# Xharlie/BtcDet

Hardware: AMD Instinct MI355X
Metric: scenes/s fwd+bwd KITTI-Car bs=2/GPU (BtcDet hot path) (higher is better)
Workload: dtype f32

## Files before the change

btcdet_amd/csrc/conv_wgrad_x.hip:

```cpp
#include <type_traits>
#include <utility>

#include "conv_tile.h"

typedef short s16x4 __attribute__((ext_vector_type(4)));
typedef short s16x8 __attribute__((ext_vector_type(8)));
typedef unsigned u32x4 __attribute__((ext_vector_type(4)));

namespace {

constexpr int TMX = 64;
#define X_RECORDS 0xFFFFFF00u
#define X_ABSENT 0xFFFFFFF0u

template <int RS>
__device__ __forceinline__ bf16x8 frag_tr(const char* p) {
  typedef __attribute__((address_space(3))) s16x4* lds_p;
  const s16x4 a = __builtin_amdgcn_ds_read_tr16_b64_v4i16((lds_p)p);
  const s16x4 b = __builtin_amdgcn_ds_read_tr16_b64_v4i16((lds_p)(p + 16 * RS));
  const s16x8 v = __builtin_shufflevector(a, b, 0, 1, 2, 3, 4, 5, 6, 7);
  return __builtin_bit_cast(bf16x8, v);
}

template <int N, typename F, int... I>
__device__ __forceinline__ void static_for_impl(F&& f, std::integer_sequence<int, I...>) {
  (f(std::integral_constant<int, I>{}), ...);
}
template <int N, typename F>
__device__ __forceinline__ void static_for(F&& f) {
  static_for_impl<N>(f, std::make_integer_sequence<int, N>{});
}

template <int MT, int NT, int KB, int PH, int MODE, int DEPTH>
__global__ __launch_bounds__(256) void conv_wgrad_x(const void* __restrict__ gsrc, const void* __restrict__ csrc,
                                                    const int32_t* __restrict__ nbr, const int32_t* __restrict__ order, int n_rows, int K,
                                                    int Cg_all, int Cc_all, float* __restrict__ part, int swap) {
  constexpr int Cg = MT * 16, Cc = NT * 16;
  const int n_cblk = (Cc_all + Cc - 1) / Cc;
  const int cg0 = ((int)blockIdx.z / n_cblk) * Cg, cc0 = ((int)blockIdx.z % n_cblk) * Cc;
  constexpr int NPL = MODE ? 3 : 1;
  constexpr int RS = Cg * 2 + 16;
  constexpr int IMG = TMX * RS;
  constexpr int ITEM = KB * NPL * IMG;
  constexpr int TPP = KB * MT * NT / 4;
  static_assert(KB * MT * NT % 4 == 0, "phase tiles must split evenly over the 4 waves");
  static_assert(4 % NT == 0, "a wave's tiles must share one column block");
  constexpr int NOFF = PH * KB;
  constexpr int NV = (TMX * NOFF + 255) / 256;
  extern __shared__ __attribute__((aligned(16))) char smem[];
  char* As = smem;
  constexpr int RING = (DEPTH == 2 && PH == 1) ? 4 : 3;
  int32_t* s_nbr = (int32_t*)(As + 2 * ITEM);
  constexpr int RROW = DEPTH == 2 ? RING + 1 : RING;
  int32_t* s_row = s_nbr + RING * TMX * NOFF;

  const int tid = threadIdx.x, lane = tid & 63, wave = tid >> 6, g4 = lane >> 4, t16 = lane & 15;
  const int kg0 = blockIdx.y * NOFF;
  const int n_tiles = (n_rows + TMX - 1) / TMX;
  const int nt_wg = ((int)blockIdx.x < n_tiles) ? (n_tiles - 1 - (int)blockIdx.x) / (int)gridDim.x + 1 : 0;
  const int bcol = cc0 + (wave % NT) * 16 + t16;
  const bool bvalid = bcol < Cc_all;
  const int lane_off = (4 * g4 + (t16 >> 2)) * RS + (t16 & 3) * 8;

  constexpr int NC = MODE ? 3 : 1;
  f32x4 acc[NC][PH * TPP];
#pragma unroll
  for (int c = 0; c < NC; ++c)
#pragma unroll
    for (int t = 0; t < PH * TPP; ++t) acc[c][t] = (f32x4){0.f, 0.f, 0.f, 0.f};

  const __amdgpu_buffer_rsrc_t rg = __builtin_amdgcn_make_buffer_rsrc((void*)gsrc, 0, X_RECORDS, 0x00020000);
  const __amdgpu_buffer_rsrc_t rc = __builtin_amdgcn_make_buffer_rsrc((void*)csrc, 0, X_RECORDS, 0x00020000);
  int nv[NV], nrow = -1;
  auto load_map = [&](int i) {
    const int row0 = (blockIdx.x + i * gridDim.x) * TMX;
    if (tid < TMX) nrow = (row0 + tid < n_rows) ? (order ? order[row0 + tid] : row0 + tid) : -1;
#pragma unroll
    for (int u = 0; u < NV; ++u) {
      const int e = u * 256 + tid, r = e / NOFF, o = e - r * NOFF;
      int v = -1;
      if (e < TMX * NOFF && row0 + r < n_rows && kg0 + o < K) {
        const int gr = order ? order[row0 + r] : row0 + r;
        v = nbr[(long long)gr * K + kg0 + o];
      }
      nv[u] = v;
    }
  };
  auto store_map = [&](int i) {
    int32_t* dn = s_nbr + (i % RING) * TMX * NOFF;
#pragma unroll
    for (int u = 0; u < NV; ++u) {
      const int e = u * 256 + tid;
      if (e < TMX * NOFF) dn[e] = nv[u];
    }
    if (tid < TMX) s_row[(i % RROW) * TMX + tid] = nrow;
  };

  auto load_rows = [&](int i) {
    const int row0 = (blockIdx.x + i * gridDim.x) * TMX;
    if (tid < TMX) nrow = (row0 + tid < n_rows) ? (order ? order[row0 + tid] : row0 + tid) : -1;
  };
  auto store_rows = [&](int i) {
    if (tid < TMX) s_row[(i % RROW) * TMX + tid] = nrow;
  };
  auto load_map2 = [&](int i) {
    const int32_t* rw = s_row + (i % RROW) * TMX;
#pragma unroll
    for (int u = 0; u < NV; ++u) {
      const int e = u * 256 + tid, r = e / NOFF, o = e - r * NOFF;
      int v = -1;
      if (e < TMX * NOFF && kg0 + o < K) {
        const int gr = rw[r];
        if (gr >= 0) v = nbr[(long long)gr * K + kg0 + o];
      }
      nv[u] = v;
    }
  };
  auto store_map2 = [&](int i) {
    int32_t* dn = s_nbr + (i % RING) * TMX * NOFF;
#pragma unroll
    for (int u = 0; u < NV; ++u) {
      const int e = u * 256 + tid;
      if (e < TMX * NOFF) dn[e] = nv[u];
    }
  };

  float bnf[MODE ? 16 : 1];
  unsigned short bnh[MODE ? 1 : 16];
  bf16x8 bh[2], bm[MODE ? 2 : 1], bl[MODE ? 2 : 1];
  auto load_b = [&](int i) {
    const int32_t* rows = s_row + (i % RROW) * TMX + 4 * g4;
    int gr[16];
#pragma unroll
    for (int u = 0; u < 16; ++u) gr[u] = rows[(u >> 2) * 16 + (u & 3)];
#pragma unroll
    for (int u = 0; u < 16; ++u) {
      const unsigned off = (gr[u] >= 0 && bvalid) ? ((unsigned)gr[u] * (unsigned)Cc_all + (unsigned)bcol) * (MODE ? 4u : 2u) : X_ABSENT;
      if (MODE) bnf[u] = __uint_as_float(__builtin_amdgcn_raw_buffer_load_b32(rc, off, 0, 0));
      else bnh[u] = __builtin_amdgcn_raw_buffer_load_b16(rc, off, 0, 0);
    }
  };
  auto take_b = [&]() {
#pragma unroll
    for (int s = 0; s < 2; ++s) {
      uint4 h, m, l;
      if (MODE) {
        btc_split3(bnf[8 * s + 0], bnf[8 * s + 1], h.x, m.x, l.x);
        btc_split3(bnf[8 * s + 2], bnf[8 * s + 3], h.y, m.y, l.y);
        btc_split3(bnf[8 * s + 4], bnf[8 * s + 5], h.z, m.z, l.z);
        btc_split3(bnf[8 * s + 6], bnf[8 * s + 7], h.w, m.w, l.w);
        bm[s] = __builtin_bit_cast(bf16x8, m);
        bl[s] = __builtin_bit_cast(bf16x8, l);
      } else {
        h.x = (unsigned)bnh[8 * s + 0] | ((unsigned)bnh[8 * s + 1] << 16);
        h.y = (unsigned)bnh[8 * s + 2] | ((unsigned)bnh[8 * s + 3] << 16);
        h.z = (unsigned)bnh[8 * s + 4] | ((unsigned)bnh[8 * s + 5] << 16);
        h.w = (unsigned)bnh[8 * s + 6] | ((unsigned)bnh[8 * s + 7] << 16);
      }
      bh[s] = __builtin_bit_cast(bf16x8, h);
    }
  };

  constexpr int UPR = MODE ? MT * 4 : MT * 2;
  constexpr int NU = (KB * TMX * UPR + 255) / 256;
  uint4 gq[DEPTH][NU];
  auto load_g = [&](int i, int p, auto set_c) {
    constexpr int SET = decltype(set_c)::value;
    const int32_t* mp = s_nbr + (i % RING) * TMX * NOFF + p * KB;
    int jj[NU];
#pragma unroll
    for (int u = 0; u < NU; ++u) {
      const int e = u * 256 + tid, r = (e / UPR) % TMX, kb = e / (UPR * TMX);
      jj[u] = (e < KB * TMX * UPR) ? mp[r * NOFF + kb] : -1;
    }
#pragma unroll
    for (int u = 0; u < NU; ++u) {
      const int c = (u * 256 + tid) % UPR;
      const unsigned off = jj[u] >= 0 ? ((unsigned)jj[u] * (unsigned)Cg_all + (unsigned)cg0) * (MODE ? 4u : 2u) + (unsigned)c * 16u : X_ABSENT;
      const u32x4 v = __builtin_amdgcn_raw_buffer_load_b128(rg, off, 0, 0);
      gq[SET][u] = make_uint4(v.x, v.y, v.z, v.w);
    }
  };
  auto store_g = [&](int buf, auto set_c) {
    constexpr int SET = decltype(set_c)::value;
    char* A = As + buf * ITEM;
#pragma unroll
    for (int u = 0; u < NU; ++u) {
      const int e = u * 256 + tid, c = e % UPR, r = (e / UPR) % TMX, kb = e / (UPR * TMX);
      if (e < KB * TMX * UPR) {
        char* d = A + kb * NPL * IMG + r * RS;
        if (MODE) {
          uint2 h, m, l;
          btc_split3(__uint_as_float(gq[SET][u].x), __uint_as_float(gq[SET][u].y), h.x, m.x, l.x);
          btc_split3(__uint_as_float(gq[SET][u].z), __uint_as_float(gq[SET][u].w), h.y, m.y, l.y);
          *reinterpret_cast<uint2*>(d + c * 8) = h;
          *reinterpret_cast<uint2*>(d + IMG + c * 8) = m;
          *reinterpret_cast<uint2*>(d + 2 * IMG + c * 8) = l;
        } else {
          *reinterpret_cast<uint4*>(d + c * 16) = gq[SET][u];
        }
      }
    }
  };

  typedef std::integral_constant<int, 0> Set0;
  typedef std::integral_constant<int, DEPTH - 1> Set1;
  if (nt_wg > 0 && DEPTH == 1) {
    load_map(0);
    store_map(0);
    if (nt_wg > 1) {
      load_map(1);
      store_map(1);
    }
    __syncthreads();
    load_b(0);
    load_g(0, 0, Set0{});
  }
  if (nt_wg > 0 && DEPTH == 2) {
    for (int j = 0; j < RROW - 1 && j < nt_wg; ++j) {
      load_rows(j);
      store_rows(j);
    }
    __syncthreads();
    for (int j = 0; j < RING - 1 && j < nt_wg; ++j) {
      load_map2(j);
      store_map2(j);
    }
    __syncthreads();
    load_b(0);
    load_g(0, 0, Set0{});
    if (PH > 1) load_g(0, 1, Set1{});
    else if (nt_wg > 1) load_g(1, 0, Set1{});
  }
  int buf = 0;
  auto products = [&](auto p_c) {
    constexpr int p = decltype(p_c)::value;
    constexpr int STEPS = 2 * TPP;
    const char* A = As + buf * ITEM + lane_off;
    bf16x8 fh[2], fm[MODE ? 2 : 1], fl[MODE ? 2 : 1];
    auto read_step = [&](int t, int w) {
      const int q = t >> 1, s2 = t & 1, l = q * 4 + wave;
      const int mt = (l / NT) % MT, kb = l / (NT * MT);
      const char* ap = A + kb * NPL * IMG + mt * 32 + 32 * s2 * RS;
      fh[w] = frag_tr<RS>(ap);
      if (MODE) {
        fm[MODE ? w : 0] = frag_tr<RS>(ap + IMG);
        fl[MODE ? w : 0] = frag_tr<RS>(ap + 2 * IMG);
      }
    };
    read_step(0, 0);
#pragma unroll
    for (int t = 0; t < STEPS; ++t) {
      const int q = t >> 1, s2 = t & 1, w = t & 1;
      if (t + 1 < STEPS) read_step(t + 1, w ^ 1);
      const bf16x8 ah = fh[w];
      if (MODE) {
        const bf16x8 am = fm[MODE ? w : 0], al = fl[MODE ? w : 0];
        f32x4 c2 = acc[NC - 1][p * TPP + q], c1 = acc[NC > 1 ? 1 : 0][p * TPP + q], c0 = acc[0][p * TPP + q];
        c2 = __builtin_amdgcn_mfma_f32_16x16x32_bf16(al, bh[s2], c2, 0, 0, 0);
        c1 = __builtin_amdgcn_mfma_f32_16x16x32_bf16(am, bh[s2], c1, 0, 0, 0);
        c0 = __builtin_amdgcn_mfma_f32_16x16x32_bf16(ah, bh[s2], c0, 0, 0, 0);
        c2 = __builtin_amdgcn_mfma_f32_16x16x32_bf16(ah, bl[MODE ? s2 : 0], c2, 0, 0, 0);
        c1 = __builtin_amdgcn_mfma_f32_16x16x32_bf16(ah, bm[MODE ? s2 : 0], c1, 0, 0, 0);
        c2 = __builtin_amdgcn_mfma_f32_16x16x32_bf16(am, bm[MODE ? s2 : 0], c2, 0, 0, 0);
        acc[NC - 1][p * TPP + q] = c2;
        acc[NC > 1 ? 1 : 0][p * TPP + q] = c1;
        acc[0][p * TPP + q] = c0;
      } else {
        acc[0][p * TPP + q] = __builtin_amdgcn_mfma_f32_16x16x32_bf16(ah, bh[s2], acc[0][p * TPP + q], 0, 0, 0);
      }
    }
  };
  if (DEPTH == 1) {
    for (int i = 0; i < nt_wg; ++i) {
      static_for<PH>([&](auto p_c) {
        constexpr int p = decltype(p_c)::value;
        store_g(buf, Set0{});
        if (p == 0) take_b();
        if (PH > 1 ? (p == 1 && i + 2 < nt_wg) : (i >= 1 && i + 1 < nt_wg)) store_map(PH > 1 ? i + 2 : i + 1);
        __syncthreads();
        if (p + 1 < PH) {
          load_g(i, p + 1, Set0{});
        } else if (i + 1 < nt_wg) {
          load_b(i + 1);
          load_g(i + 1, 0, Set0{});
        }
        if (PH > 1 ? (p == 0 && i + 2 < nt_wg) : (i + 2 < nt_wg)) load_map(i + 2);
        products(p_c);
        buf ^= 1;
      });
    }
  } else if (PH > 1) {
    for (int i = 0; i < nt_wg; ++i) {
      static_for<PH>([&](auto p_c) {
        constexpr int p = decltype(p_c)::value;
        typedef std::integral_constant<int, (p & 1) ? DEPTH - 1 : 0> Set;
        store_g(buf, Set{});
        if (p == 0) take_b();
        if (p == 1 && i + 2 < nt_wg) store_map2(i + 2);
        if (p == 1 && i + 3 < nt_wg) store_rows(i + 3);
        __syncthreads();
        if (p == PH - 2 && i + 1 < nt_wg) load_b(i + 1);
        if (p == 0 && i + 3 < nt_wg) load_rows(i + 3);
        if (p == 0 && i + 2 < nt_wg) load_map2(i + 2);
        if (p + 2 < PH) load_g(i, p + 2, Set{});
        else if (i + 1 < nt_wg) load_g(i + 1, p + 2 - PH, Set{});
        products(p_c);
        buf ^= 1;
      });
    }
  } else {
    auto tile = [&](int i, auto set_c) {
      store_g(buf, set_c);
      take_b();
      if (i >= 1 && i + 2 < nt_wg) store_map2(i + 2);
      if (i >= 1 && i + 3 < nt_wg) store_rows(i + 3);
      __syncthreads();
      if (i + 1 < nt_wg) load_b(i + 1);
      if (i + 4 < nt_wg) load_rows(i + 4);
      if (i + 3 < nt_wg) load_map2(i + 3);
      if (i + 2 < nt_wg) load_g(i + 2, 0, set_c);
      products(std::integral_constant<int, 0>{});
      buf ^= 1;
    };
    for (int i = 0; i < nt_wg; i += 2) {
      tile(i, Set0{});
      if (i + 1 < nt_wg) tile(i + 1, Set1{});
    }
  }
  float* P = part + (size_t)blockIdx.x * K * Cg_all * Cc_all;
#pragma unroll
  for (int p = 0; p < PH; ++p)
#pragma unroll
    for (int q = 0; q < TPP; ++q) {
      const int l = q * 4 + wave;
      const int nt = l % NT, mt = (l / NT) % MT, kb = l / (NT * MT);
      const int k = kg0 + p * KB + kb;
      const int co = cc0 + nt * 16 + t16;
      if (k >= K || co >= Cc_all) continue;
#pragma unroll
      for (int r = 0; r < 4; ++r) {
        const int ci = cg0 + mt * 16 + g4 * 4 + r;
        float v = acc[0][p * TPP + q][r];
        if (MODE) v = v + (acc[NC > 1 ? 1 : 0][p * TPP + q][r] + acc[NC - 1][p * TPP + q][r]);
        if (!swap) P[((size_t)k * Cg_all + ci) * Cc_all + co] = v;
        else P[((size_t)k * Cc_all + co) * Cg_all + ci] = v;
      }
    }
}

template <int MT, int NT, int KB, int PH, int MODE, int DEPTH>
size_t lds_x() {
  constexpr int NPL = MODE ? 3 : 1;
  constexpr int RING = (DEPTH == 2 && PH == 1) ? 4 : 3;
  constexpr int RROW = DEPTH == 2 ? RING + 1 : RING;
  return (size_t)2 * KB * NPL * TMX * (MT * 32 + 16) + (size_t)(RING * TMX * PH * KB + RROW * TMX) * sizeof(int32_t);
}

template <int MT, int NT, int KB, int PH, int MODE, int DEPTH>
void launch_x(dim3 grid, hipStream_t stream, const void* g, const void* c, const int32_t* map, const int32_t* ord, int rows, int K, int cg_all,
              int cc_all, float* part, int swap) {
  static BtcPerDeviceOnce once;
  btc_once_per_device(once, [] {
    (void)hipFuncSetAttribute((const void*)conv_wgrad_x<MT, NT, KB, PH, MODE, DEPTH>, hipFuncAttributeMaxDynamicSharedMemorySize, 160 * 1024);
  });
  conv_wgrad_x<MT, NT, KB, PH, MODE, DEPTH><<<grid, 256, lds_x<MT, NT, KB, PH, MODE, DEPTH>(), stream>>>(g, c, map, ord, rows, K, cg_all, cc_all, part, swap);
}

struct XShape {
  int mt, nt, kb, ph;
};
const XShape X_BF16[] = {{4, 4, 1, 4}, {4, 2, 1, 8}, {2, 4, 2, 4}, {3, 2, 2, 4}, {2, 2, 2, 8}, {2, 1, 2, 8}, {1, 2, 4, 4}, {1, 1, 4, 4}};
const XShape X_SPLIT[] = {{4, 4, 1, 2}, {4, 2, 1, 4}, {2, 4, 2, 2}, {3, 2, 2, 2}, {2, 2, 2, 4}, {2, 1, 2, 8}, {1, 2, 2, 8}};

const XShape* find_shape(int mode, int cg_all, int cc_all) {
  if (cg_all <= 0 || cc_all <= 0 || (cg_all & 15)) return nullptr;
  const XShape* tab = mode ? X_SPLIT : X_BF16;
  const int n = mode ? (int)(sizeof(X_SPLIT) / sizeof(XShape)) : (int)(sizeof(X_BF16) / sizeof(XShape));
  const int nt_want = cc_all <= 16 ? 1 : (cc_all <= 32 ? 2 : 4);
  for (int nt = nt_want; nt >= 1; nt >>= 1)
    for (int i = 0; i < n; ++i) {
      if (tab[i].nt != nt) continue;
      const int cg = tab[i].mt * 16;
      if (cg_all % cg != 0 || (tab[i].mt == 3 && cg_all != 48)) continue;
      return tab + i;
    }
  return nullptr;
}

}

bool btc_wgrad_x_supported(int mode, int K, int cg, int cc) {
  if (K > 64 || K < 1) return false;
  return find_shape(mode, cg, cc) != nullptr;
}

int btc_wgrad_x_plan(int mode, int rows, int K, int cg, int cc, int* S, int* ph, int* z) {
  const XShape* sh = find_shape(mode, cg, cc);
  const int t_wgs = btc_tune_get(BTC_TUNE_WGRAD_WGS);
  const int wgs = t_wgs ? t_wgs : 512;
  const int n_tiles = btc_cdiv(rows, TMX);
  const int nz = (cg / (sh->mt * 16)) * btc_cdiv(cc, sh->nt * 16);
  int p = sh->ph;
  if (p > 1 && (long long)n_tiles * btc_cdiv(K, sh->kb * p) * nz < 3LL * wgs) p >>= 1;
  const int groups = btc_cdiv(K, sh->kb * p);
  int s = wgs / (groups * nz);
  if (s > n_tiles / 2) s = n_tiles / 2;
  if (s < 1) s = 1;
  *S = s;
  *ph = p;
  if (z) *z = nz;
  return groups;
}

int btc_launch_wgrad_x(int mode, const void* g, const void* c, const int32_t* map, const int32_t* ord, int rows, int K, int cg, int cc, float* part,
                       int swap, hipStream_t stream) {
  const XShape* sh = find_shape(mode, cg, cc);
  BTC_CHECK_ARG(sh != nullptr && K <= 64, "btc_launch_wgrad_x: unsupported shape %d x %d (mode %d)", cg, cc, mode);
  int S = 1, ph = 1, nz = 1;
  const int groups = btc_wgrad_x_plan(mode, rows, K, cg, cc, &S, &ph, &nz);
  dim3 grid(S, groups, nz);
  const int t_depth = btc_tune_get(BTC_TUNE_WGRAD_X_DEPTH);
  const bool shallow = t_depth ? t_depth == 1 : mode == 1;
#define X2(MT_, NT_, KB_, PH_, MODE_)                                                                            \
  do {                                                                                                           \
    if (shallow) launch_x<MT_, NT_, KB_, PH_, MODE_, 1>(grid, stream, g, c, map, ord, rows, K, cg, cc, part, swap);  \
    else launch_x<MT_, NT_, KB_, PH_, MODE_, 2>(grid, stream, g, c, map, ord, rows, K, cg, cc, part, swap);          \
  } while (0)
#define X(MT_, NT_, KB_, PH_, MODE_)                                \
  do {                                                              \
    if (ph == PH_) X2(MT_, NT_, KB_, PH_, MODE_);                   \
    else X2(MT_, NT_, KB_, (PH_ / 2), MODE_);                       \
  } while (0)
  const int mt = sh->mt, nt = sh->nt;
  if (mode == 0) {
    if (mt == 1 && nt == 1) X(1, 1, 4, 4, 0);
    else if (mt == 2 && nt == 1) X(2, 1, 2, 8, 0);
    else if (mt == 1 && nt == 2) X(1, 2, 4, 4, 0);
    else if (mt == 2 && nt == 2) X(2, 2, 2, 8, 0);
    else if (mt == 3 && nt == 2) X(3, 2, 2, 4, 0);
    else if (mt == 2 && nt == 4) X(2, 4, 2, 4, 0);
    else if (mt == 4 && nt == 2) X(4, 2, 1, 8, 0);
    else X(4, 4, 1, 4, 0);
  } else {
    if (mt == 2 && nt == 1) X(2, 1, 2, 8, 1);
    else if (mt == 1 && nt == 2) X(1, 2, 2, 8, 1);
    else if (mt == 2 && nt == 2) X(2, 2, 2, 4, 1);
    else if (mt == 3 && nt == 2) X(3, 2, 2, 2, 1);
    else if (mt == 2 && nt == 4) X(2, 4, 2, 2, 1);
    else if (mt == 4 && nt == 2) X(4, 2, 1, 4, 1);
    else X(4, 4, 1, 2, 1);
  }
#undef X
#undef X2
  BTC_LAUNCH_CHECK();
  return BTC_OK;
}
```

Baseline: 589.3.

## Add compacted pair-queue walk to sparse conv weight-grad kernel

```diff
diff --git a/btcdet_amd/csrc/conv_wgrad_x.hip b/btcdet_amd/csrc/conv_wgrad_x.hip
--- a/btcdet_amd/csrc/conv_wgrad_x.hip
+++ b/btcdet_amd/csrc/conv_wgrad_x.hip
@@ -12,6 +12,10 @@
 constexpr int TMX = 64;
 #define X_RECORDS 0xFFFFFF00u
 #define X_ABSENT 0xFFFFFFF0u
+constexpr int QCAP = 256;
+constexpr int X_FILL_NUM = 3, X_FILL_DEN = 10;
+#define X_INL __attribute__((always_inline))
+enum { X_WALK_AUTO = 0, X_WALK_TILES = 2, X_WALK_PAIRS = 3 };
 
 template <int RS>
 __device__ __forceinline__ bf16x8 frag_tr(const char* p) {
@@ -31,10 +35,15 @@
   static_for_impl<N>(f, std::make_integer_sequence<int, N>{});
 }
 
-template <int MT, int NT, int KB, int PH, int MODE, int DEPTH>
-__global__ __launch_bounds__(256) void conv_wgrad_x(const void* __restrict__ gsrc, const void* __restrict__ csrc,
+template <int MT, int NT, int KB, int PH, int MODE>
+constexpr bool pair_auto() {
+  return MODE == 1 && KB == 1;
+}
+
+template <int MT, int NT, int KB, int PH, int MODE, int DEPTH, bool PW>
+__global__ __launch_bounds__(256, (PW && pair_auto<MT, NT, KB, PH, MODE>()) ? 2 : 1) void conv_wgrad_x(const void* __restrict__ gsrc, const void* __restrict__ csrc,
                                                     const int32_t* __restrict__ nbr, const int32_t* __restrict__ order, int n_rows, int K,
-                                                    int Cg_all, int Cc_all, float* __restrict__ part, int swap) {
+                                                    int Cg_all, int Cc_all, float* __restrict__ part, int swap, int walk) {
   constexpr int Cg = MT * 16, Cc = NT * 16;
   const int n_cblk = (Cc_all + Cc - 1) / Cc;
   const int cg0 = ((int)blockIdx.z / n_cblk) * Cg, cc0 = ((int)blockIdx.z % n_cblk) * Cc;
@@ -53,6 +62,10 @@
   int32_t* s_nbr = (int32_t*)(As + 2 * ITEM);
   constexpr int RROW = DEPTH == 2 ? RING + 1 : RING;
   int32_t* s_row = s_nbr + RING * TMX * NOFF;
+  int32_t* s_qg = s_row + RROW * TMX;
+  int32_t* s_qr = s_qg + NOFF * QCAP;
+  int32_t* s_tot = s_qr + NOFF * QCAP;
+  int32_t* s_red = s_tot + 2 * NOFF;
 
   const int tid = threadIdx.x, lane = tid & 63, wave = tid >> 6, g4 = lane >> 4, t16 = lane & 15;
   const int kg0 = blockIdx.y * NOFF;
@@ -72,7 +85,7 @@
   const __amdgpu_buffer_rsrc_t rg = __builtin_amdgcn_make_buffer_rsrc((void*)gsrc, 0, X_RECORDS, 0x00020000);
   const __amdgpu_buffer_rsrc_t rc = __builtin_amdgcn_make_buffer_rsrc((void*)csrc, 0, X_RECORDS, 0x00020000);
   int nv[NV], nrow = -1;
-  auto load_map = [&](int i) {
+  auto load_map = [&](int i) X_INL {
     const int row0 = (blockIdx.x + i * gridDim.x) * TMX;
     if (tid < TMX) nrow = (row0 + tid < n_rows) ? (order ? order[row0 + tid] : row0 + tid) : -1;
 #pragma unroll
@@ -86,7 +99,7 @@
       nv[u] = v;
     }
   };
-  auto store_map = [&](int i) {
+  auto store_map = [&](int i) X_INL {
     int32_t* dn = s_nbr + (i % RING) * TMX * NOFF;
 #pragma unroll
     for (int u = 0; u < NV; ++u) {
@@ -96,14 +109,14 @@
     if (tid < TMX) s_row[(i % RROW) * TMX + tid] = nrow;
   };
 
-  auto load_rows = [&](int i) {
+  auto load_rows = [&](int i) X_INL {
     const int row0 = (blockIdx.x + i * gridDim.x) * TMX;
     if (tid < TMX) nrow = (row0 + tid < n_rows) ? (order ? order[row0 + tid] : row0 + tid) : -1;
   };
-  auto store_rows = [&](int i) {
+  auto store_rows = [&](int i) X_INL {
     if (tid < TMX) s_row[(i % RROW) * TMX + tid] = nrow;
   };
-  auto load_map2 = [&](int i) {
+  auto load_map2 = [&](int i) X_INL {
     const int32_t* rw = s_row + (i % RROW) * TMX;
 #pragma unroll
     for (int u = 0; u < NV; ++u) {
@@ -116,7 +129,7 @@
       nv[u] = v;
     }
   };
-  auto store_map2 = [&](int i) {
+  auto store_map2 = [&](int i) X_INL {
     int32_t* dn = s_nbr + (i % RING) * TMX * NOFF;
 #pragma unroll
     for (int u = 0; u < NV; ++u) {
@@ -125,54 +138,56 @@
     }
   };
 
-  float bnf[MODE ? 16 : 1];
-  unsigned short bnh[MODE ? 1 : 16];
-  bf16x8 bh[2], bm[MODE ? 2 : 1], bl[MODE ? 2 : 1];
-  auto load_b = [&](int i) {
+  constexpr bool KBW = (MT * NT) % 4 != 0;
+  constexpr int NB = KBW ? TPP : KB;
+  float bnf[MODE ? NB : 1][MODE ? 16 : 1];
+  unsigned short bnh[MODE ? 1 : NB][MODE ? 1 : 16];
+  bf16x8 bh[NB][2], bm[MODE ? NB : 1][MODE ? 2 : 1], bl[MODE ? NB : 1][MODE ? 2 : 1];
+  auto fetch_b = [&](auto bs_c, const int (&gr)[16]) {
+    constexpr int BS = decltype(bs_c)::value;
+#pragma unroll
+    for (int u = 0; u < 16; ++u) {
+      const unsigned off = (gr[u] >= 0 && bvalid) ? ((unsigned)gr[u] * (unsigned)Cc_all + (unsigned)bcol) * (MODE ? 4u : 2u) : X_ABSENT;
+      if (MODE) bnf[MODE ? BS : 0][MODE ? u : 0] = __uint_as_float(__builtin_amdgcn_raw_buffer_load_b32(rc, off, 0, 0));
+      else bnh[MODE ? 0 : BS][MODE ? 0 : u] = __builtin_amdgcn_raw_buffer_load_b16(rc, off, 0, 0);
+    }
+  };
+  auto load_b = [&](int i) X_INL {
     const int32_t* rows = s_row + (i % RROW) * TMX + 4 * g4;
     int gr[16];
 #pragma unroll
     for (int u = 0; u < 16; ++u) gr[u] = rows[(u >> 2) * 16 + (u & 3)];
-#pragma unroll
-    for (int u = 0; u < 16; ++u) {
-      const unsigned off = (gr[u] >= 0 && bvalid) ? ((unsigned)gr[u] * (unsigned)Cc_all + (unsigned)bcol) * (MODE ? 4u : 2u) : X_ABSENT;
-      if (MODE) bnf[u] = __uint_as_float(__builtin_amdgcn_raw_buffer_load_b32(rc, off, 0, 0));
-      else bnh[u] = __builtin_amdgcn_raw_buffer_load_b16(rc, off, 0, 0);
-    }
-  };
-  auto take_b = [&]() {
+    fetch_b(std::integral_constant<int, 0>{}, gr);
+  };
+  auto take_b = [&](auto bs_c) X_INL {
+    constexpr int BS = decltype(bs_c)::value;
+    constexpr int BF = MODE ? BS : 0, BH = MODE ? 0 : BS;
 #pragma unroll
     for (int s = 0; s < 2; ++s) {
       uint4 h, m, l;
       if (MODE) {
-        btc_split3(bnf[8 * s + 0], bnf[8 * s + 1], h.x, m.x, l.x);
-        btc_split3(bnf[8 * s + 2], bnf[8 * s + 3], h.y, m.y, l.y);
-        btc_split3(bnf[8 * s + 4], bnf[8 * s + 5], h.z, m.z, l.z);
-        btc_split3(bnf[8 * s + 6], bnf[8 * s + 7], h.w, m.w, l.w);
-        bm[s] = __builtin_bit_cast(bf16x8, m);
-        bl[s] = __builtin_bit_cast(bf16x8, l);
+        btc_split3(bnf[BF][MODE ? 8 * s + 0 : 0], bnf[BF][MODE ? 8 * s + 1 : 0], h.x, m.x, l.x);
+        btc_split3(bnf[BF][MODE ? 8 * s + 2 : 0], bnf[BF][MODE ? 8 * s + 3 : 0], h.y, m.y, l.y);
+        btc_split3(bnf[BF][MODE ? 8 * s + 4 : 0], bnf[BF][MODE ? 8 * s + 5 : 0], h.z, m.z, l.z);
+        btc_split3(bnf[BF][MODE ? 8 * s + 6 : 0], bnf[BF][MODE ? 8 * s + 7 : 0], h.w, m.w, l.w);
+        bm[BF][MODE ? s : 0] = __builtin_bit_cast(bf16x8, m);
+        bl[BF][MODE ? s : 0] = __builtin_bit_cast(bf16x8, l);
       } else {
-        h.x = (unsigned)bnh[8 * s + 0] | ((unsigned)bnh[8 * s + 1] << 16);
-        h.y = (unsigned)bnh[8 * s + 2] | ((unsigned)bnh[8 * s + 3] << 16);
-        h.z = (unsigned)bnh[8 * s + 4] | ((unsigned)bnh[8 * s + 5] << 16);
-        h.w = (unsigned)bnh[8 * s + 6] | ((unsigned)bnh[8 * s + 7] << 16);
-      }
-      bh[s] = __builtin_bit_cast(bf16x8, h);
-    }
-  };
+        h.x = (unsigned)bnh[BH][MODE ? 0 : 8 * s + 0] | ((unsigned)bnh[BH][MODE ? 0 : 8 * s + 1] << 16);
+        h.y = (unsigned)bnh[BH][MODE ? 0 : 8 * s + 2] | ((unsigned)bnh[BH][MODE ? 0 : 8 * s + 3] << 16);
+        h.z = (unsigned)bnh[BH][MODE ? 0 : 8 * s + 4] | ((unsigned)bnh[BH][MODE ? 0 : 8 * s + 5] << 16);
+        h.w = (unsigned)bnh[BH][MODE ? 0 : 8 * s + 6] | ((unsigned)bnh[BH][MODE ? 0 : 8 * s + 7] << 16);
+      }
+      bh[BS][s] = __builtin_bit_cast(bf16x8, h);
+    }
+  };
+  typedef std::integral_constant<int, 0> Slot0;
 
   constexpr int UPR = MODE ? MT * 4 : MT * 2;
   constexpr int NU = (KB * TMX * UPR + 255) / 256;
   uint4 gq[DEPTH][NU];
-  auto load_g = [&](int i, int p, auto set_c) {
+  auto fetch_g = [&](const int (&jj)[NU], auto set_c) {
     constexpr int SET = decltype(set_c)::value;
-    const int32_t* mp = s_nbr + (i % RING) * TMX * NOFF + p * KB;
-    int jj[NU];
-#pragma unroll
-    for (int u = 0; u < NU; ++u) {
-      const int e = u * 256 + tid, r = (e / UPR) % TMX, kb = e / (UPR * TMX);
-      jj[u] = (e < KB * TMX * UPR) ? mp[r * NOFF + kb] : -1;
-    }
 #pragma unroll
     for (int u = 0; u < NU; ++u) {
       const int c = (u * 256 + tid) % UPR;
@@ -181,7 +196,17 @@
       gq[SET][u] = make_uint4(v.x, v.y, v.z, v.w);
     }
   };
-  auto store_g = [&](int buf, auto set_c) {
+  auto load_g = [&](int i, int p, auto set_c) X_INL {
+    const int32_t* mp = s_nbr + (i % RING) * TMX * NOFF + p * KB;
+    int jj[NU];
+#pragma unroll
+    for (int u = 0; u < NU; ++u) {
+      const int e = u * 256 + tid, r = (e / UPR) % TMX, kb = e / (UPR * TMX);
+      jj[u] = (e < KB * TMX * UPR) ? mp[r * NOFF + kb] : -1;
+    }
+    fetch_g(jj, set_c);
+  };
+  auto store_g = [&](int buf, auto set_c) X_INL {
     constexpr int SET = decltype(set_c)::value;
     char* A = As + buf * ITEM;
 #pragma unroll
@@ -213,8 +238,6 @@
       store_map(1);
     }
     __syncthreads();
-    load_b(0);
-    load_g(0, 0, Set0{});
   }
   if (nt_wg > 0 && DEPTH == 2) {
     for (int j = 0; j < RROW - 1 && j < nt_wg; ++j) {
@@ -227,18 +250,48 @@
       store_map2(j);
     }
     __syncthreads();
+  }
+  bool pairs = PW && walk == X_WALK_PAIRS;
+  if (PW && walk == X_WALK_AUTO && nt_wg > 0) {
+    const int nt2 = nt_wg > 1 ? 2 : 1;
+    int np = 0;
+    for (int j = 0; j < nt2; ++j)
+#pragma unroll
+      for (int u = 0; u < NV; ++u) {
+        const int e = u * 256 + tid;
+        const bool pr = e < TMX * NOFF && s_nbr[j * TMX * NOFF + (e < TMX * NOFF ? e : 0)] >= 0;
+        np += __popcll(__ballot(pr));
+      }
+    if (lane == 0) s_red[wave] = np;
+    __syncthreads();
+    np = s_red[0] + s_red[1] + s_red[2] + s_red[3];
+    int rows2 = n_rows - (int)blockIdx.x * TMX;
+    rows2 = rows2 < TMX ? rows2 : TMX;
+    if (nt2 > 1) {
+      const int r1 = n_rows - ((int)blockIdx.x + (int)gridDim.x) * TMX;
+      rows2 += r1 < TMX ? r1 : TMX;
+    }
+    const int offs = K - kg0 < NOFF ? K - kg0 : NOFF;
+    pairs = (long long)np * X_FILL_DEN < (long long)X_FILL_NUM * rows2 * offs;
+  }
+  if (nt_wg > 0 && DEPTH == 1 && !pairs) {
+    load_b(0);
+    load_g(0, 0, Set0{});
+  }
+  if (nt_wg > 0 && DEPTH == 2 && !pairs) {
     load_b(0);
     load_g(0, 0, Set0{});
     if (PH > 1) load_g(0, 1, Set1{});
     else if (nt_wg > 1) load_g(1, 0, Set1{});
   }
   int buf = 0;
-  auto products = [&](auto p_c) {
+  auto products = [&](auto p_c, auto pair_c) X_INL {
     constexpr int p = decltype(p_c)::value;
+    constexpr bool PAIR = decltype(pair_c)::value;
     constexpr int STEPS = 2 * TPP;
     const char* A = As + buf * ITEM + lane_off;
     bf16x8 fh[2], fm[MODE ? 2 : 1], fl[MODE ? 2 : 1];
-    auto read_step = [&](int t, int w) {
+    auto read_step = [&](int t, int w) X_INL {
       const int q = t >> 1, s2 = t & 1, l = q * 4 + wave;
       const int mt = (l / NT) % MT, kb = l / (NT * MT);
       const char* ap = A + kb * NPL * IMG + mt * 32 + 32 * s2 * RS;
@@ -252,31 +305,125 @@
 #pragma unroll
     for (int t = 0; t < STEPS; ++t) {
       const int q = t >> 1, s2 = t & 1, w = t & 1;
+      const int bs = !PAIR ? 0 : (KBW ? q : q / (MT * NT / 4 > 0 ? MT * NT / 4 : 1));
+      const int bsm = MODE ? bs : 0;
       if (t + 1 < STEPS) read_step(t + 1, w ^ 1);
       const bf16x8 ah = fh[w];
       if (MODE) {
         const bf16x8 am = fm[MODE ? w : 0], al = fl[MODE ? w : 0];
         f32x4 c2 = acc[NC - 1][p * TPP + q], c1 = acc[NC > 1 ? 1 : 0][p * TPP + q], c0 = acc[0][p * TPP + q];
-        c2 = __builtin_amdgcn_mfma_f32_16x16x32_bf16(al, bh[s2], c2, 0, 0, 0);
-        c1 = __builtin_amdgcn_mfma_f32_16x16x32_bf16(am, bh[s2], c1, 0, 0, 0);
-        c0 = __builtin_amdgcn_mfma_f32_16x16x32_bf16(ah, bh[s2], c0, 0, 0, 0);
-        c2 = __builtin_amdgcn_mfma_f32_16x16x32_bf16(ah, bl[MODE ? s2 : 0], c2, 0, 0, 0);
-        c1 = __builtin_amdgcn_mfma_f32_16x16x32_bf16(ah, bm[MODE ? s2 : 0], c1, 0, 0, 0);
-        c2 = __builtin_amdgcn_mfma_f32_16x16x32_bf16(am, bm[MODE ? s2 : 0], c2, 0, 0, 0);
+        c2 = __builtin_amdgcn_mfma_f32_16x16x32_bf16(al, bh[bs][s2], c2, 0, 0, 0);
+        c1 = __builtin_amdgcn_mfma_f32_16x16x32_bf16(am, bh[bs][s2], c1, 0, 0, 0);
+        c0 = __builtin_amdgcn_mfma_f32_16x16x32_bf16(ah, bh[bs][s2], c0, 0, 0, 0);
+        c2 = __builtin_amdgcn_mfma_f32_16x16x32_bf16(ah, bl[bsm][MODE ? s2 : 0], c2, 0, 0, 0);
+        c1 = __builtin_amdgcn_mfma_f32_16x16x32_bf16(ah, bm[bsm][MODE ? s2 : 0], c1, 0, 0, 0);
+        c2 = __builtin_amdgcn_mfma_f32_16x16x32_bf16(am, bm[bsm][MODE ? s2 : 0], c2, 0, 0, 0);
         acc[NC - 1][p * TPP + q] = c2;
         acc[NC > 1 ? 1 : 0][p * TPP + q] = c1;
         acc[0][p * TPP + q] = c0;
       } else {
-        acc[0][p * TPP + q] = __builtin_amdgcn_mfma_f32_16x16x32_bf16(ah, bh[s2], acc[0][p * TPP + q], 0, 0, 0);
-      }
-    }
-  };
-  if (DEPTH == 1) {
+        acc[0][p * TPP + q] = __builtin_amdgcn_mfma_f32_16x16x32_bf16(ah, bh[bs][s2], acc[0][p * TPP + q], 0, 0, 0);
+      }
+    }
+  };
+  if (PW && pairs) {
+    int q_tot = 0, q_taken = 0, etot[(NOFF + 3) / 4];
+#pragma unroll
+    for (int m = 0; m < (NOFF + 3) / 4; ++m) etot[m] = 0;
+    auto enqueue = [&](int i, int par) X_INL {
+      const int32_t* mp = s_nbr + (i % RING) * TMX * NOFF + lane * NOFF;
+      const int wr = s_row[(i % RROW) * TMX + lane];
+#pragma unroll
+      for (int m = 0; m < (NOFF + 3) / 4; ++m) {
+        const int o = wave + 4 * m;
+        if (o < NOFF) {
+          const int v = mp[o];
+          const unsigned long long mask = __ballot(v >= 0);
+          if (v >= 0) {
+            const int pos = (etot[m] + __popcll(mask & ((1ull << lane) - 1ull))) & (QCAP - 1);
+            s_qg[o * QCAP + pos] = v;
+            s_qr[o * QCAP + pos] = wr;
+          }
+          etot[m] += __popcll(mask);
+          if (lane == 0) s_tot[par * NOFF + o] = etot[m];
+        }
+      }
+    };
+    auto load_item = [&](int pn) X_INL {
+      const int avail = q_tot - q_taken, nk_l = avail < TMX ? avail : TMX;
+      int base[KB], nk[KB];
+#pragma unroll
+      for (int kb = 0; kb < KB; ++kb) {
+        base[kb] = __builtin_amdgcn_readlane(q_taken, pn * KB + kb);
+        nk[kb] = __builtin_amdgcn_readlane(nk_l, pn * KB + kb);
+      }
+      static_for<NB>([&](auto bs_c) X_INL {
+        constexpr int BS = decltype(bs_c)::value;
+        const int kbs = KBW ? (BS * 4 + wave) / (MT * NT) : BS;
+        int b0 = 0, nn = 0;
+#pragma unroll
+        for (int kb = 0; kb < KB; ++kb)
+          if (kb == kbs) b0 = base[kb], nn = nk[kb];
+        const int32_t* qr = s_qr + (pn * KB + kbs) * QCAP;
+        int gr[16];
+#pragma unroll
+        for (int u = 0; u < 16; ++u) {
+          const int sl = (u >> 2) * 16 + (u & 3) + 4 * g4;
+          gr[u] = sl < nn ? qr[(b0 + sl) & (QCAP - 1)] : -1;
+        }
+        fetch_b(bs_c, gr);
+      });
+      int jj[NU];
+#pragma unroll
+      for (int u = 0; u < NU; ++u) {
+        const int e = u * 256 + tid, r = (e / UPR) % TMX, kbe = e / (UPR * TMX);
+        int b0 = 0, nn = 0;
+#pragma unroll
+        for (int kb = 0; kb < KB; ++kb)
+          if (kb == kbe) b0 = base[kb], nn = nk[kb];
+        jj[u] = (e < KB * TMX * UPR && r < nn) ? s_qg[(pn * KB + kbe) * QCAP + ((b0 + r) & (QCAP - 1))] : -1;
+      }
+      fetch_g(jj, Set0{});
+      if (lane / KB == pn) q_taken += nk_l;
+    };
+    int pp = -1, nxt = 0, par = 0;
+    unsigned ready = 0;
+    for (;;) {
+      const bool enq = ready == 0 && nxt < nt_wg;
+      if (pp >= 0) {
+        store_g(buf, Set0{});
+        static_for<NB>([&](auto bs_c) X_INL { take_b(bs_c); });
+      }
+      if (enq) {
+        if (nxt >= 1 && nxt + 1 < nt_wg) store_map(nxt + 1);
+        if (nxt + 2 < nt_wg) load_map(nxt + 2);
+        enqueue(nxt, par);
+        ++nxt;
+      }
+      __syncthreads();
+      if (enq) q_tot = lane < NOFF ? s_tot[par * NOFF + lane] : 0;
+      ready = (unsigned)__ballot(lane < NOFF && q_tot - q_taken >= TMX);
+      if (ready == 0 && nxt >= nt_wg) ready = (unsigned)__ballot(lane < NOFF && q_tot - q_taken > 0);
+      const int pn = ready ? (__ffs(ready) - 1) / KB : -1;
+      if (pn >= 0) load_item(pn);
+      if (pp >= 0) {
+        static_for<PH>([&](auto q_c) X_INL {
+          if (pp == decltype(q_c)::value) products(q_c, std::true_type{});
+        });
+        buf ^= 1;
+      }
+      pp = pn;
+      par ^= 1;
+      ready = (unsigned)__ballot(lane < NOFF && q_tot - q_taken >= TMX);
+      if (ready == 0 && nxt >= nt_wg) ready = (unsigned)__ballot(lane < NOFF && q_tot - q_taken > 0);
+      if (pp < 0 && ready == 0 && nxt >= nt_wg) break;
+    }
+  } else if (DEPTH == 1) {
     for (int i = 0; i < nt_wg; ++i) {
-      static_for<PH>([&](auto p_c) {
+      static_for<PH>([&](auto p_c) X_INL {
         constexpr int p = decltype(p_c)::value;
         store_g(buf, Set0{});
-        if (p == 0) take_b();
+        if (p == 0) take_b(Slot0{});
         if (PH > 1 ? (p == 1 && i + 2 < nt_wg) : (i >= 1 && i + 1 < nt_wg)) store_map(PH > 1 ? i + 2 : i + 1);
         __syncthreads();
         if (p + 1 < PH) {
@@ -286,17 +433,17 @@
           load_g(i + 1, 0, Set0{});
         }
         if (PH > 1 ? (p == 0 && i + 2 < nt_wg) : (i + 2 < nt_wg)) load_map(i + 2);
-        products(p_c);
+        products(p_c, std::false_type{});
         buf ^= 1;
       });
     }
   } else if (PH > 1) {
     for (int i = 0; i < nt_wg; ++i) {
-      static_for<PH>([&](auto p_c) {
+      static_for<PH>([&](auto p_c) X_INL {
         constexpr int p = decltype(p_c)::value;
         typedef std::integral_constant<int, (p & 1) ? DEPTH - 1 : 0> Set;
         store_g(buf, Set{});
-        if (p == 0) take_b();
+        if (p == 0) take_b(Slot0{});
         if (p == 1 && i + 2 < nt_wg) store_map2(i + 2);
         if (p == 1 && i + 3 < nt_wg) store_rows(i + 3);
         __syncthreads();
@@ -305,14 +452,14 @@
         if (p == 0 && i + 2 < nt_wg) load_map2(i + 2);
         if (p + 2 < PH) load_g(i, p + 2, Set{});
         else if (i + 1 < nt_wg) load_g(i + 1, p + 2 - PH, Set{});
-        products(p_c);
+        products(p_c, std::false_type{});
         buf ^= 1;
       });
     }
   } else {
-    auto tile = [&](int i, auto set_c) {
+    auto tile = [&](int i, auto set_c) X_INL {
       store_g(buf, set_c);
-      take_b();
+      take_b(Slot0{});
       if (i >= 1 && i + 2 < nt_wg) store_map2(i + 2);
       if (i >= 1 && i + 3 < nt_wg) store_rows(i + 3);
       __syncthreads();
@@ -320,7 +467,7 @@
       if (i + 4 < nt_wg) load_rows(i + 4);
       if (i + 3 < nt_wg) load_map2(i + 3);
       if (i + 2 < nt_wg) load_g(i + 2, 0, set_c);
-      products(std::integral_constant<int, 0>{});
+      products(std::integral_constant<int, 0>{}, std::false_type{});
       buf ^= 1;
     };
     for (int i = 0; i < nt_wg; i += 2) {
@@ -356,15 +503,28 @@
   constexpr int RROW = DEPTH == 2 ? RING + 1 : RING;
   return (size_t)2 * KB * NPL * TMX * (MT * 32 + 16) + (size_t)(RING * TMX * PH * KB + RROW * TMX) * sizeof(int32_t);
 }
+template <int KB, int PH>
+size_t lds_pairs() {
+  return (size_t)(2 * PH * KB * QCAP + 2 * PH * KB + 4) * sizeof(int32_t);
+}
+
+template <int MT, int NT, int KB, int PH, int MODE, int DEPTH, bool PW>
+void launch_xw(dim3 grid, size_t lds, hipStream_t stream, const void* g, const void* c, const int32_t* map, const int32_t* ord, int rows, int K,
+               int cg_all, int cc_all, float* part, int swap, int walk) {
+  static BtcPerDeviceOnce once;
+  btc_once_per_device(once, [] {
+    (void)hipFuncSetAttribute((const void*)conv_wgrad_x<MT, NT, KB, PH, MODE, DEPTH, PW>, hipFuncAttributeMaxDynamicSharedMemorySize, 160 * 1024);
+  });
+  conv_wgrad_x<MT, NT, KB, PH, MODE, DEPTH, PW><<<grid, 256, lds, stream>>>(g, c, map, ord, rows, K, cg_all, cc_all, part, swap, walk);
+}
 
 template <int MT, int NT, int KB, int PH, int MODE, int DEPTH>
 void launch_x(dim3 grid, hipStream_t stream, const void* g, const void* c, const int32_t* map, const int32_t* ord, int rows, int K, int cg_all,
-              int cc_all, float* part, int swap) {
-  static BtcPerDeviceOnce once;
-  btc_once_per_device(once, [] {
-    (void)hipFuncSetAttribute((const void*)conv_wgrad_x<MT, NT, KB, PH, MODE, DEPTH>, hipFuncAttributeMaxDynamicSharedMemorySize, 160 * 1024);
-  });
-  conv_wgrad_x<MT, NT, KB, PH, MODE, DEPTH><<<grid, 256, lds_x<MT, NT, KB, PH, MODE, DEPTH>(), stream>>>(g, c, map, ord, rows, K, cg_all, cc_all, part, swap);
+              int cc_all, float* part, int swap, int walk) {
+  const size_t lds = lds_x<MT, NT, KB, PH, MODE, DEPTH>(), ldsp = lds + lds_pairs<KB, PH>();
+  if (walk == X_WALK_AUTO && !pair_auto<MT, NT, KB, PH, MODE>()) walk = X_WALK_TILES;
+  if (walk == X_WALK_TILES) launch_xw<MT, NT, KB, PH, MODE, DEPTH, false>(grid, lds, stream, g, c, map, ord, rows, K, cg_all, cc_all, part, swap, walk);
+  else launch_xw<MT, NT, KB, PH, MODE, DEPTH, true>(grid, ldsp, stream, g, c, map, ord, rows, K, cg_all, cc_all, part, swap, walk);
 }
 
 struct XShape {
@@ -422,10 +582,12 @@
   dim3 grid(S, groups, nz);
   const int t_depth = btc_tune_get(BTC_TUNE_WGRAD_X_DEPTH);
   const bool shallow = t_depth ? t_depth == 1 : mode == 1;
+  const int t_walk = btc_tune_get(BTC_TUNE_WGRAD_X);
+  const int walk = t_walk == 2 ? X_WALK_TILES : (t_walk == 3 ? X_WALK_PAIRS : X_WALK_AUTO);
 #define X2(MT_, NT_, KB_, PH_, MODE_)                                                                            \
   do {                                                                                                           \
-    if (shallow) launch_x<MT_, NT_, KB_, PH_, MODE_, 1>(grid, stream, g, c, map, ord, rows, K, cg, cc, part, swap);  \
-    else launch_x<MT_, NT_, KB_, PH_, MODE_, 2>(grid, stream, g, c, map, ord, rows, K, cg, cc, part, swap);          \
+    if (shallow) launch_x<MT_, NT_, KB_, PH_, MODE_, 1>(grid, stream, g, c, map, ord, rows, K, cg, cc, part, swap, walk);  \
+    else launch_x<MT_, NT_, KB_, PH_, MODE_, 2>(grid, stream, g, c, map, ord, rows, K, cg, cc, part, swap, walk);          \
   } while (0)
 #define X(MT_, NT_, KB_, PH_, MODE_)                                \
   do {                                                              \
```

New measurement: 597.0, median of 6. +1.3%, better.
